# Thealexbarney/VGAudio

Measured on AMD Instinct MI355X. Metric: Msamples/s encoded (GC-ADPCM, 4096 ch) at 1/2/4/8 GPUs; % HBM roofline, higher is better.
Workload: dtype int32; 1 GPU; BASELINE configs[1]: 4096 mono channels x 48 kHz x 60 s GC-ADPCM coefficient search + encode per GPU; parallelism=units sharded x1, channels_per_gpu=4096, samples_per_channel=2880000, bit_exact_channels_checked=0

## Files before the change

vgaudio_amd/csrc/gc_encode_core.hpp:

```cpp
#pragma once
#include <cstdint>

#if defined(__HIPCC__)
#define VGA_HD __host__ __device__ __forceinline__
#else
#define VGA_HD inline
#endif

#if defined(__HIP_DEVICE_COMPILE__)
#define VGA_MUL24(a, b) __mul24((a), (b))
#define VGA_OPAQUE(v) asm("" : "+v"(v))
#define VGA_OPAQUE_S(v) asm("" : "+s"(v))
static __device__ __forceinline__ uint32_t vga_square24(int e)
{
    uint32_t r;
    asm("v_mul_i32_i24 %0, %1, %1" : "=v"(r) : "v"(e));
    return r;
}
#else
#define VGA_MUL24(a, b) ((a) * (b))
#define VGA_OPAQUE(v) ((void)0)
#define VGA_OPAQUE_S(v) ((void)0)
#endif

// ... 404 lines not shown
        const int P = (HAVE_P0 && s == 0) ? P0_b : dot2_i16(h, cpair, kacc);
        uint32_t b;
        const int d = (int)sub_borrow_u32((uint32_t)in_b[s], (uint32_t)P, b);
        const int rd = NO_ROUND ? d : round_through_f32(d);
        const int u2 = (int)((uint32_t)rd + (uint32_t)bias2 + b) >> k;
        const int q2 = med3_i32(u2, q_lo, q_hi);
        if (s & 1) {
            umax = imax(imax(umax, u_prev), u2);
            umin = imin(imin(umin, u_prev), u2);
        }
        u_prev = u2;
        if (!OV_ONLY) r.q2[s] = q2;
        const int w = (P >> 11) + (int)((uint32_t)q2 << km11);
        h = sat_pack16(w_prev, w);
        w_prev = w;
        if ((s & 1) && !OV_ONLY) {
            if (WITH_SUM) {
                const uint32_t epk = pk_sub_sat_i16(xw[s >> 1], h);
                total = dot2_i16(epk, epk, total);
            } else
                r.pairs[s >> 1] = h;
        }
    }
    r.hist_pair = h;
    const int ov = imax(imax(umax - q_hi, q_lo - umin), 0);
    r.exact = pass_b_coef_ok(c0, c1) && ov <= 12383 && (((2 * ov + 1) << (k - 11)) <= 24766);
    r.total = (uint64_t)(uint32_t)total;
    r.max_overflow = ov;
    return r;
}
VGA_HD bool pass_a_is_final(int sp_a, int ov_a) { return sp_a >= 12 || ov_a <= 1; }
template <bool NO_ROUND>
VGA_HD PassOutB final_pass_pair(const uint32_t (&xw)[7], uint32_t hist, const int (&in_b)[14], int c0, int c1, int sp_a, int sp_b,
                                int P0_b, int &ov_a, int &sp2)
{
    ov_a = pass_fast_core_b<NO_ROUND, true, false, true>(xw, hist, in_b, c0, c1, sp_a, P0_b).max_overflow;
    sp2 = pass_a_is_final(sp_a, ov_a) ? sp_a : sp_b;
    return pass_fast_core_b<NO_ROUND, true, false>(xw, hist, in_b, c0, c1, sp2, P0_b);
}
struct FrameFlags { bool fin_a, bump_a, bump_b, generic, inexact, resume; };
VGA_HD FrameFlags frame_flags(int sp_a, int sp_b, int ov_a, int ov_b, bool coef_ok)
{
    FrameFlags f;
    const bool cap_a = sp_a >= 12, cap_b = sp_b >= 12;
    const int eff_a = cap_a ? 0 : ov_a, eff_b = cap_b ? 0 : ov_b;
    f.fin_a = eff_a < 2;
    f.bump_a = !cap_a && (unsigned)ov_a > 248u;
    f.bump_b = !f.fin_a && !cap_b && (unsigned)ov_b > 248u;
    f.generic = !coef_ok || f.bump_a || f.bump_b;
    f.inexact = !f.generic && (f.fin_a ? (cap_a && (unsigned)ov_a > 3u) : (cap_b && (unsigned)ov_b > 3u));
    f.resume = !f.generic && !f.fin_a && eff_b >= 2;
    return f;
}
VGA_HD void pack_frame_mod16(const int (&q)[14], int predictor, int scale_power, uint32_t &d0, uint32_t &d1)
{
    uint32_t wa = 0, wb = 0;
#if defined(__HIP_DEVICE_COMPILE__)
#pragma unroll
#endif
    for (int s = 0; s < 14; s++) {
        if (s < 6) wa = (wa << 4) | ((uint32_t)q[s] & 15u);
        else       wb = (wb << 4) | ((uint32_t)q[s] & 15u);
    }
    const uint32_t header = (uint32_t)((predictor << 4) | (scale_power & 0xF));
    d0 = bswap32((header << 24) | wa);
    d1 = bswap32(wb);
}
VGA_HD PassOutB as_pass_b(const PassOut &r)
{
    PassOutB o;
#if defined(__HIP_DEVICE_COMPILE__)
#pragma unroll
#endif
    for (int s = 0; s < 14; s++) o.q2[s] = r.q[s];
    o.total = r.total; o.max_overflow = r.max_overflow; o.hist_pair = r.hist_pair; o.exact = r.exact;
    return o;
}
constexpr uint64_t PACKED_SUM_CAP = 1ull << 28;
VGA_HD bool needs_exact_sum(uint64_t total, bool known_exact) { return !known_exact && total >= PACKED_SUM_CAP; }
VGA_HD PassOut pass_fast_core(const int (&x)[16], uint32_t hist, const int (&in2048p)[14], int c0, int c1, int scale_power)
{
    uint32_t xw[7];
    pack_row(x, xw);
    return pass_fast_core_t<false>(xw, hist, in2048p, c0, c1, scale_power);
}
VGA_HD PassOut pass_fast_core_no_round(const int (&x)[16], uint32_t hist, const int (&in2048p)[14], int c0, int c1,
                                       int scale_power)
{
    uint32_t xw[7];
    pack_row(x, xw);
    return pass_fast_core_t<false, true>(xw, hist, in2048p, c0, c1, scale_power);
}
VGA_HD PassOut pass_fast_core_wide(const int (&x)[16], uint32_t hist, const int (&in2048p)[14], int c0, int c1,
                                   int scale_power)
{
    uint32_t xw[7];
    pack_row(x, xw);
    return pass_fast_core_t<true>(xw, hist, in2048p, c0, c1, scale_power);
}
template <bool NO_ROUND>
VGA_HD PassOut pass_fast_core_exact_sum(const int (&x)[16], const int (&in2048p)[14], int c0, int c1, int scale_power)
{
    uint32_t xw[7];
    pack_row(x, xw);
    const uint32_t hist = pack16(x[0], x[1]);
    PassOut r = pass_fast_core_t<false, NO_ROUND>(xw, hist, in2048p, c0, c1, scale_power);
// ... 94 lines not shown
```

vgaudio_amd/csrc/gc_encode_kernel.hip:

```cpp
#include "common.hpp"
#include "gc_encode_core.hpp"
#include "gcadpcm_kernels.hpp"
#include "seams.hpp"

#include <cstdio>
#include <cstdlib>

namespace vga {
namespace gc {

constexpr int DPP_QUAD_XOR1 = 0xB1;
constexpr int DPP_QUAD_XOR2 = 0x4E;
constexpr int DPP_ROW_HALF_MIRROR = 0x141;
constexpr int DPP_ROW_MIRROR = 0x140;

template <int CTRL>
__device__ __forceinline__ int dpp(int v)
{
    return __builtin_amdgcn_update_dpp(0, v, CTRL, 0xF, 0xF, true);
}

__device__ __forceinline__ unsigned umin32(unsigned a, unsigned b) { return a < b ? a : b; }

template <class Op>
__device__ __forceinline__ unsigned row16_reduce(unsigned v, Op op)
{
    v = op(v, (unsigned)dpp<DPP_QUAD_XOR1>((int)v));
    v = op(v, (unsigned)dpp<DPP_QUAD_XOR2>((int)v));
    v = op(v, (unsigned)dpp<DPP_ROW_HALF_MIRROR>((int)v));
    v = op(v, (unsigned)dpp<DPP_ROW_MIRROR>((int)v));
    return v;
}


#ifdef VGA_DEBUG_TIMESTAMPS
__device__ unsigned long long g_vga_enc_ts[1 << 16];
extern "C" int vga_debug_encode_timestamps(unsigned long long *out, int n)
{
    return (int)hipMemcpyFromSymbol(out, HIP_SYMBOL(g_vga_enc_ts), (size_t)n * sizeof(unsigned long long));
}
#endif
__device__ unsigned long long g_vga_gc_stats[8];
extern "C" int vga_testing_gc_encode_stats(unsigned long long *out8, int reset)
{
    if (hipDeviceSynchronize() != hipSuccess) return -1;
    if (out8 && hipMemcpyFromSymbol(out8, HIP_SYMBOL(g_vga_gc_stats), 8 * sizeof(unsigned long long)) != hipSuccess) return -1;
#ifdef VGA_GC_STATS
    if (out8) out8[7] = 1;
#else
    if (out8) out8[7] = 0;
#endif
    if (reset) {
        const unsigned long long zero[8] = {0, 0, 0, 0, 0, 0, 0, 0};
        if (hipMemcpyToSymbol(HIP_SYMBOL(g_vga_gc_stats), zero, sizeof zero) != hipSuccess) return -1;
    }
    return 0;
}
constexpr int SW = 2;
constexpr int ENC_THREADS = 64 * (SW + 1);
#ifndef VGA_GC_ENCODER_PRIO
#define VGA_GC_ENCODER_PRIO 3
#endif
#ifndef VGA_GC_HELPER_PRIO
#define VGA_GC_HELPER_PRIO 0
#endif
template <int CPW>
struct Lay {
    static constexpr int CS = CPW * SW;
    static constexpr int TF = 64 / CS;
};
template <int CS, int TF>
struct GcTileT {
    uint32_t xw[CS][TF][8];
    int in2048p[CS][TF][16];
    uint32_t pre[CS][TF][8];
};
typedef short short2v __attribute__((ext_vector_type(2)));
struct XW7 { uint32_t v[7]; };

#define VGA_COLD __device__ __forceinline__

VGA_COLD int prescan_sequential_cold(XW7 xs, uint32_t hist, int c0, int c1)
{
    int x[16];
    unpack_row(xs.v, hist, x);
    return prescan_sequential(x, c0, c1);
}

#ifdef VGA_GC_R05_COLD
#define VGA_COLD_OPAQUE(v) ((void)0)
#else
#define VGA_COLD_OPAQUE(v) VGA_OPAQUE(v)
#endif
struct ColdState {
    uint32_t xw[7];
    int mp[14];
    uint32_t hist;
    int c0, c1, s1;
    int generic, start, drop, wide, resume;
    int bump_a, ov_a, ov_b;
};
struct ColdOut { PassOutB r; int final_sp; int fin; int sum_exact; };
__device__ __forceinline__
ColdOut encode_frame_cold(ColdState st, PassOutB r, int final_sp, int fin)
{
    uint32_t xw[7];
    int mp[14];
#pragma unroll
    for (int i = 0; i < 7; i++) xw[i] = st.xw[i];
#pragma unroll
    for (int i = 0; i < 14; i++) mp[i] = st.mp[i];
    int sum_exact = 0;
    if (st.drop) fin = 0;
    if (__any(st.generic != 0)) {
        if (st.generic) {
            int xg[16];
            unpack_row(xw, st.hist, xg);
#pragma unroll
            for (int i = 0; i < 16; i++) VGA_COLD_OPAQUE(xg[i]);
            const int start = st.start != -100 ? st.start
                                               : (st.bump_a ? apply_bumps(st.s1, st.ov_a) : apply_bumps(st.s1 + 1, st.ov_b));
            r = as_pass_b(resume_passes(xg, st.c0, st.c1, start, final_sp));
            fin = 1;
            sum_exact = 1;
        }
    }
    if (st.wide) fin = 1;
    if (__any(st.resume != 0)) {
// ... 20 lines not shown
                    r = as_pass_b(resume_passes(xg, st.c0, st.c1, sp - 1, final_sp));
                    sum_exact = 1;
                    break;
                }
                final_sp = sp;
                if (cap || r.max_overflow <= 1) break;
            }
            fin = 1;
        }
    }
    ColdOut o;
    o.r = r;
    o.final_sp = final_sp;
    o.fin = fin;
    o.sum_exact = sum_exact;
    return o;
}

template <bool REPAIR, int CPW, bool RAGGED>
__device__ __forceinline__ void gc_encode_piece(
    const int bx, const int by,
    const int16_t *__restrict__ pcm, int64_t pcm_pitch, int nch, int total_samples, const Pieces seg,
    const int16_t *__restrict__ coefs, const int16_t *__restrict__ hist1,
    const int16_t *__restrict__ hist2, uint8_t *__restrict__ adpcm, int64_t adpcm_pitch, int16_t *__restrict__ seg_state,
    const int *__restrict__ first_open, const Ragged &rg)
{
    constexpr bool repair = REPAIR;
    constexpr int CS = Lay<CPW>::CS, TF = Lay<CPW>::TF;
    using GcTile = GcTileT<CS, TF>;
    int64_t first_frame = seg.first(by);
    int repair_piece = 0;
    if (repair) {
        int k = SEAM_OPEN_LIMIT;
        for (int g = 0; g < CS; g++) {
            const int slot = bx * CS + g;
            if (slot < nch) {
                const int c = RAGGED ? rg.order[slot] : slot;
                k = first_open[c] < k ? first_open[c] : k;
            }
        }
        if (!is_open(k)) return;
        repair_piece = k;
        first_frame = seg.first(k);
    }
    const int total_wg = RAGGED ? rg.length[rg.order[bx * CS]] : total_samples;
    if (first_frame * 14 >= total_wg) return;
    const int64_t piece_samples = repair ? (int64_t)0x7fffffff : (int64_t)seg.frames(by) * 14;
    auto piece_samples_of = [&](int total) {
        const int64_t rem = (int64_t)total - first_frame * 14;
        return (int)(rem < 0 ? 0 : (rem < piece_samples ? rem : piece_samples));
    };
    pcm += first_frame * 14;
    adpcm += first_frame * 8;
    __shared__ GcTile s_tile[2];
    __shared__ int4 s_out[2][CS][TF][4];
    __shared__ int s_ncold[SW];
    const int tid = threadIdx.x;
    const int wave = tid >> 6;
    const bool helper = wave == SW;
    const int lane = tid & 63;
    constexpr int LPC = 64 / CPW;
    int grp = helper ? lane / TF : wave * CPW + lane / LPC;
    const int l16 = lane & (LPC - 1);
    const int hfr = lane % TF;
    const int slot_raw = bx * CS + grp;
    const bool live = slot_raw < nch;
    const int slot = live ? slot_raw : nch - 1;
    const int ch = RAGGED ? rg.order[slot] : slot;
    const int16_t *src = pcm + (RAGGED ? rg.pcm_off[ch] : (int64_t)ch * pcm_pitch);
    uint8_t *dst = adpcm + (RAGGED ? rg.adpcm_off[ch] : (int64_t)ch * adpcm_pitch);

    const int sample_count = piece_samples_of(RAGGED ? rg.length[ch] : total_samples);
    const int full_frames = sample_count / 14;
    const int tail = sample_count - full_frames * 14;
    const int frames = full_frames + (tail ? 1 : 0);
    const int frames_wg = RAGGED ? (piece_samples_of(total_wg) + 13) / 14 : frames;
    const int tiles = (frames_wg + TF - 1) / TF;

    if (helper) {
        __builtin_amdgcn_s_setprio(VGA_GC_HELPER_PRIO);
        uint32_t cpk[8];
#pragma unroll
        for (int p = 0; p < 8; p++)
            cpk[p] = (uint32_t)(uint16_t)coefs[ch * 16 + 2 * p + 1] | ((uint32_t)(uint16_t)coefs[ch * 16 + 2 * p] << 16);
        auto prepare = [&](int tile) {
            const int fr = RAGGED ? imax(imin(tile * TF + hfr, frames - 1), 0) : imin(tile * TF + hfr, frames - 1);
            int in[14];
            uint32_t w[7];
            if (fr < full_frames) {
                const uint32_t *p32 = reinterpret_cast<const uint32_t *>(src + (int64_t)fr * 14);
#pragma unroll
                for (int i = 0; i < 7; i++) w[i] = p32[i];
#pragma unroll
                for (int i = 0; i < 7; i++) {
                    in[2 * i] = (int)(int16_t)(w[i] & 0xFFFF);
                    in[2 * i + 1] = (int)w[i] >> 16;
                }
            } else {
#pragma unroll
                for (int s = 0; s < 14; s++) in[s] = (s < tail) ? (int)src[(int64_t)fr * 14 + s] : 0;
#pragma unroll
                for (int i = 0; i < 7; i++) w[i] = (uint32_t)(in[2 * i] & 0xFFFF) | ((uint32_t)in[2 * i + 1] << 16);
            }
            GcTile &T = s_tile[tile & 1];
            uint4 *xr = reinterpret_cast<uint4 *>(&T.xw[grp][hfr][0]);
            xr[0] = make_uint4(w[0], w[1], w[2], w[3]);
            xr[1] = make_uint4(w[4], w[5], w[6], 0u);
            int4 *qr = reinterpret_cast<int4 *>(&T.in2048p[grp][hfr][0]);
            qr[0] = make_int4(pass_b_row(in[0]), pass_b_row(in[1]), pass_b_row(in[2]), pass_b_row(in[3]));
            qr[1] = make_int4(pass_b_row(in[4]), pass_b_row(in[5]), pass_b_row(in[6]), pass_b_row(in[7]));
            qr[2] = make_int4(pass_b_row(in[8]), pass_b_row(in[9]), pass_b_row(in[10]), pass_b_row(in[11]));
            qr[3] = make_int4(pass_b_row(in[12]), pass_b_row(in[13]), 0, 0);
            uint32_t pair[12];
#pragma unroll
            for (int k = 0; k < 12; k++)
                pair[k] = (k & 1) ? __builtin_amdgcn_alignbit(w[(k + 1) / 2], w[(k - 1) / 2], 16) : w[k / 2];
            uint32_t pre[8];
#pragma unroll
            for (int p = 0; p < 8; p++) {
                int dmax = 0, dmin = 0;
#ifdef VGA_GC_ABLATE_HELPER_PRESCAN
                dmax = in[2 + p] & 1023;
                dmin = -(in[3 + p] & 1023);
#else
#pragma unroll
                for (int k = 0; k < 12; k++) {
                    const int predicted = div2048(__builtin_amdgcn_sdot2(__builtin_bit_cast(short2v, pair[k]),
                                                                         __builtin_bit_cast(short2v, cpk[p]), 0, false));
                    const int d = in[k + 2] - predicted;
                    dmax = imax(dmax, d);
                    dmin = imin(dmin, d);
                }
#endif
                pre[p] = (uint32_t)(clamp16i(dmax) & 0xFFFF) | ((uint32_t)clamp16i(dmin) << 16);
            }
            uint4 *pr = reinterpret_cast<uint4 *>(&T.pre[grp][hfr][0]);
            pr[0] = make_uint4(pre[0], pre[1], pre[2], pre[3]);
            pr[1] = make_uint4(pre[4], pre[5], pre[6], pre[7]);
        };
        auto flush = [&](int tile) {
            const int fr = tile * TF + hfr;
            if (!live || fr >= frames) return;
            const int4 *rec = &s_out[tile & 1][grp][hfr][0];
            const int4 r0 = rec[0], r1 = rec[1], r2 = rec[2], r3 = rec[3];
            const int q[14] = {r0.x, r0.y, r0.z, r0.w, r1.x, r1.y, r1.z, r1.w, r2.x, r2.y, r2.z, r2.w, r3.x, r3.y};
            uint2 v;
            pack_frame_mod16(q, r3.z, r3.w, v.x, v.y);
            if (fr < full_frames) {
                *reinterpret_cast<uint2 *>(dst + (int64_t)fr * 8) = v;
            } else {
                const int nbytes = (tail + 2 + 1) / 2;
                const uint64_t both = ((uint64_t)v.y << 32) | v.x;
                for (int b = 0; b < nbytes; b++) dst[(int64_t)fr * 8 + b] = (uint8_t)(both >> (8 * b));
            }
        };
        if (tiles > 0) prepare(0);
        __syncthreads();
        for (int tile = 0; tile < tiles; tile++) {
            if (tile + 1 < tiles) prepare(tile + 1);
            if (tile > 0) flush(tile - 1);
            __syncthreads();
        }
        if (tiles > 0) flush(tiles - 1);
        return;
    }

    __builtin_amdgcn_s_setprio(VGA_GC_ENCODER_PRIO);
    int p = CPW == 4 ? l16 >> 1 : l16;
    const bool cand_b = CPW == 4 && (l16 & 1) != 0;
    const int c0 = coefs[ch * 16 + 2 * p];
    const int c1 = coefs[ch * 16 + 2 * p + 1];
    const bool coef_ok = pass_b_coef_ok(c0, c1);
    int h0 = hist2 ? hist2[ch] : 0;
    int h1 = hist1 ? hist1[ch] : 0;
    if (repair) {
        h0 = seg_state[((int64_t)(repair_piece - 1) * nch + ch) * 2];
        h1 = seg_state[((int64_t)(repair_piece - 1) * nch + ch) * 2 + 1];
    } else if (by > 0 && (!RAGGED || frames > 0)) {
        h0 = src[-2];
        h1 = src[-1];
    }
    uint32_t hpk = pack16(h0, h1);

    if (lane == 0) s_ncold[wave] = 0;
    struct Row { uint32_t xw[7]; int mp[14]; uint32_t pre; };
    auto read_row = [&](const GcTile &T, int j, Row &R) {
        const uint4 *xr = reinterpret_cast<const uint4 *>(&T.xw[grp][j][0]);
        const uint4 a0 = xr[0], a1 = xr[1];
        asm volatile("" ::"v"(a1.w));
        uint32_t *xw = R.xw;
        xw[0] = a0.x; xw[1] = a0.y; xw[2] = a0.z; xw[3] = a0.w; xw[4] = a1.x; xw[5] = a1.y; xw[6] = a1.z;
        const int4 *qr = reinterpret_cast<const int4 *>(&T.in2048p[grp][j][0]);
        const int4 e0 = qr[0], e1 = qr[1], e2 = qr[2], e3 = qr[3];
        asm volatile("" ::"v"(e3.z), "v"(e3.w));
        int *mp = R.mp;
        mp[0] = e0.x; mp[1] = e0.y; mp[2] = e0.z; mp[3] = e0.w; mp[4] = e1.x; mp[5] = e1.y; mp[6] = e1.z; mp[7] = e1.w;
        mp[8] = e2.x; mp[9] = e2.y; mp[10] = e2.z; mp[11] = e2.w; mp[12] = e3.x; mp[13] = e3.y;
        R.pre = T.pre[grp][j][p];
    };
    auto pack = [](const uint32_t (&xw)[7]) {
        XW7 xs;
#pragma unroll
        for (int i = 0; i < 7; i++) xs.v[i] = xw[i];
        return xs;
    };
    const uint32_t cpk = pack16(c1, c0);
    auto wide_total = [&](const uint32_t (&xw)[7], const int (&mp)[14], int sp) -> uint64_t {
        int row[14];
#pragma unroll
        for (int i = 0; i < 14; i++) row[i] = mp[i] - PASS_B_OFF;
        return pass_fast_core_wide(xw, hpk, row, c0, c1, sp).total;
    };
    const bool head_numer = __builtin_amdgcn_ballot_w64(!coef_ok) == 0;
    auto prescan_head = [&](const Row &R, int &d0, int &d1, int &P0) __attribute__((always_inline)) {
        P0 = predicted_b(hpk, cpk);
        if (__builtin_expect(head_numer, 1)) {
            d0 = head_distance_numer_b(R.mp[0], P0);
            d1 = head_distance_numer_b(R.mp[1], predicted_b(__builtin_amdgcn_alignbit(R.xw[0], hpk, 16), cpk));
        } else {
            d0 = pair_lo(R.xw[0]) - div2048(dot2_i16_wrap(hpk, cpk));
            d1 = pair_hi(R.xw[0]) - div2048(dot2_i16_wrap(__builtin_amdgcn_alignbit(R.xw[0], hpk, 16), cpk));
        }
    };
    auto first_scale = [&](const Row &R, int d0, int d1) __attribute__((always_inline)) -> int {
        const int dmax = imax(imax((int)(int16_t)(R.pre & 0xFFFF), d0), d1);
        const int dmin = imin(imin((int)R.pre >> 16, d0), d1);
        int sum, pos;
        int s1 = first_scale_power_nt(dmax, dmin, sum, pos);
        if (__builtin_expect(__builtin_amdgcn_ballot_w64(sum == 0) != 0, 0)) {
            if (sum == 0 && first_scale_tie(pos)) s1 = first_scale_power_from_md(prescan_sequential_cold(pack(R.xw), hpk, c0, c1));
        }
        return s1;
    };

    auto encode_frame = [&](Row &R, int buf, int j, bool upd) {
        const uint32_t (&xw)[7] = R.xw;
        int s1, P0;
        {
            int d0, d1;
            prescan_head(R, d0, d1, P0);
            s1 = first_scale(R, d0, d1);
        }
        int final_sp = imin(s1 + (cand_b ? 1 : 0), 12);
        const bool at_cap = final_sp >= 12;
        const unsigned ov_limit = at_cap ? 3u : 248u;
        PassOutB r = pass_fast_core_b<false, true>(xw, hpk, R.mp, c0, c1, final_sp, P0);
        const bool rare = !coef_ok || (!at_cap && (unsigned)r.max_overflow > ov_limit);
        const int eff = at_cap ? 0 : r.max_overflow;
        const int eff_other = dpp<DPP_QUAD_XOR1>(eff);
        bool fin = eff < 2 && (eff_other | (cand_b ? 0 : 2)) >= 2;
        const bool resume = !cand_b && imin(eff, eff_other) >= 2;
        const bool inexact = fin && at_cap && (unsigned)r.max_overflow > ov_limit;
        constexpr unsigned SAT = (1u << 28) - 1;
        auto argmin32 = [&](const PassOutB &r, bool fin, bool &sat) __attribute__((always_inline)) -> int {
            const unsigned tot = umin32((unsigned)(r.total >> 32) ? SAT : (unsigned)r.total, SAT);
            const unsigned key = fin ? ((tot << 4) | (unsigned)l16) : 0xFFFFFFFFu;
            const unsigned best = row16_reduce(key, [](unsigned a, unsigned b) { return a < b ? a : b; });
            sat = __any((best >> 4) >= SAT);
            return (int)(best & 15u);
        };
        auto argmin64 = [&](uint64_t total, bool fin) __attribute__((always_inline)) -> int {
            uint64_t key = fin ? ((total << 4) | (uint64_t)l16) : ~0ull;
#define VGA_MIN64_STAGE(CTRL)                                                          \
            {                                                                          \
                const unsigned olo = (unsigned)dpp<CTRL>((int)(uint32_t)key);          \
                const unsigned ohi = (unsigned)dpp<CTRL>((int)(uint32_t)(key >> 32));  \
                const uint64_t okey = ((uint64_t)ohi << 32) | olo;                     \
                key = okey < key ? okey : key;                                         \
            }
            VGA_MIN64_STAGE(DPP_QUAD_XOR1)
            VGA_MIN64_STAGE(DPP_QUAD_XOR2)
            VGA_MIN64_STAGE(DPP_ROW_HALF_MIRROR)
            VGA_MIN64_STAGE(DPP_ROW_MIRROR)
#undef VGA_MIN64_STAGE
            return (int)(key & 15u);
        };
        auto commit = [&](const PassOutB &r, int final_sp, int winner) __attribute__((always_inline)) {
            const bool won = l16 == winner;
            const unsigned pay = row16_reduce(won ? r.hist_pair : 0u,
                                              [](unsigned a, unsigned b) { return a | b; });
            if (won) {
                int4 *rec = &s_out[buf][grp][j][0];
                rec[0] = make_int4(r.q2[0], r.q2[1], r.q2[2], r.q2[3]);
                rec[1] = make_int4(r.q2[4], r.q2[5], r.q2[6], r.q2[7]);
                rec[2] = make_int4(r.q2[8], r.q2[9], r.q2[10], r.q2[11]);
                rec[3] = make_int4(r.q2[12], r.q2[13], p, final_sp);
            }
            if (!RAGGED || upd) hpk = pay;
        };
        bool sat = false;
        const int winner32 = argmin32(r, fin && !inexact, sat);
        if (__builtin_expect(__any(rare || resume || inexact) || sat, 0)) {
#ifdef VGA_GC_STATS
            if (lane == 0) atomicAdd(&s_ncold[wave], 1);
#endif
            ColdState st;
#pragma unroll
            for (int i = 0; i < 7; i++) st.xw[i] = xw[i];
#pragma unroll
            for (int i = 0; i < 14; i++) st.mp[i] = R.mp[i];
            st.hist = hpk;
            st.c0 = c0; st.c1 = c1; st.s1 = s1;
            const bool redo = __any(rare);
            st.generic = redo && !cand_b; st.start = s1 - 1; st.drop = redo && cand_b;
            st.wide = !redo && inexact; st.resume = !redo && resume;
            st.bump_a = 0; st.ov_a = 0; st.ov_b = 0;
            const ColdOut o = encode_frame_cold(st, r, final_sp, fin);
            bool sat2 = false;
            int winner = argmin32(o.r, o.fin != 0, sat2);
            if (sat2) {
                uint64_t total = o.r.total;
                if (o.fin != 0 && needs_exact_sum(total, o.sum_exact != 0))
                    total = wide_total(xw, R.mp, o.final_sp);
                winner = argmin64(total, o.fin != 0);
            }
            commit(o.r, o.final_sp, winner);
        } else
            commit(r, final_sp, winner32);
    };

    auto encode_frame8 = [&](Row &R, int buf, int j, bool upd) {
        const uint32_t (&xw)[7] = R.xw;
        int s1, P0;
        {
            int d0, d1;
            prescan_head(R, d0, d1, P0);
            s1 = first_scale(R, d0, d1);
        }
        const int sp_a = imin(s1, 12), sp_b = imin(s1 + 1, 12);
        PassOutB r;
        int ov_a, sp2;
#ifdef VGA_GC_NO_FAST_PASSES
        bool short_passes = false;
#else
        bool short_passes = !__any(sp_b > 9);
#endif
        if (short_passes) {
            r = final_pass_pair<true>(xw, hpk, R.mp, c0, c1, sp_a, sp_b, P0, ov_a, sp2);
            const bool trusted = !coef_ok || (pass_no_round_is_exact(sp_a, ov_a) && pass_no_round_is_exact(sp2, r.max_overflow));
            short_passes = !__any(!trusted);
        }
        if (!short_passes) r = final_pass_pair<false>(xw, hpk, R.mp, c0, c1, sp_a, sp_b, P0, ov_a, sp2);
        const int ov_2 = r.max_overflow;
        const FrameFlags ff = frame_flags(sp_a, sp_b, ov_a, ov_2, coef_ok);
        const bool bump_a = ff.bump_a, generic = ff.generic, inexact = ff.inexact;
#ifdef VGA_GC_ABLATE_THIRD_TRIPS
        const bool resume = false;
#else
        const bool resume = ff.resume;
#endif
        r.total = error_sum_pairs(xw, r.pairs);
        r.exact = true;
        const int final_sp = sp2;
        constexpr unsigned SAT = (1u << 28) - 1;
        auto argmin32 = [&](const PassOutB &r, bool fin, bool &sat) __attribute__((always_inline)) -> int {
            const unsigned tot = umin32((unsigned)(r.total >> 32) ? SAT : (unsigned)r.total, SAT);
            unsigned key = fin ? ((tot << 3) | (unsigned)p) : 0xFFFFFFFFu;
            key = umin32(key, (unsigned)dpp<DPP_QUAD_XOR1>((int)key));
            key = umin32(key, (unsigned)dpp<DPP_QUAD_XOR2>((int)key));
            key = umin32(key, (unsigned)dpp<DPP_ROW_HALF_MIRROR>((int)key));
            sat = __any((key >> 3) >= SAT);
            return (int)(key & 7u);
        };
        auto argmin64 = [&](uint64_t total, bool fin) __attribute__((always_inline)) -> int {
            uint64_t key = fin ? ((total << 3) | (uint64_t)p) : ~0ull;
#define VGA_MIN64_STAGE(CTRL)                                                          \
            {                                                                          \
                const unsigned olo = (unsigned)dpp<CTRL>((int)(uint32_t)key);          \
                const unsigned ohi = (unsigned)dpp<CTRL>((int)(uint32_t)(key >> 32));  \
                const uint64_t okey = ((uint64_t)ohi << 32) | olo;                     \
                key = okey < key ? okey : key;                                         \
            }
            VGA_MIN64_STAGE(DPP_QUAD_XOR1)
            VGA_MIN64_STAGE(DPP_QUAD_XOR2)
            VGA_MIN64_STAGE(DPP_ROW_HALF_MIRROR)
#undef VGA_MIN64_STAGE
            return (int)(key & 7u);
        };
        auto commit = [&](const PassOutB &r, int final_sp, int winner) __attribute__((always_inline)) {
            const bool won = p == winner;
            unsigned pay = won ? r.hist_pair : 0u;
            pay |= (unsigned)dpp<DPP_QUAD_XOR1>((int)pay);
            pay |= (unsigned)dpp<DPP_QUAD_XOR2>((int)pay);
            pay |= (unsigned)dpp<DPP_ROW_HALF_MIRROR>((int)pay);
            if (won) {
                int4 *rec = &s_out[buf][grp][j][0];
                rec[0] = make_int4(r.q2[0], r.q2[1], r.q2[2], r.q2[3]);
                rec[1] = make_int4(r.q2[4], r.q2[5], r.q2[6], r.q2[7]);
                rec[2] = make_int4(r.q2[8], r.q2[9], r.q2[10], r.q2[11]);
                rec[3] = make_int4(r.q2[12], r.q2[13], p, final_sp);
            }
            if (!RAGGED || upd) hpk = pay;
        };
        bool sat = false;
        const int winner32 = argmin32(r, !(generic || resume || inexact), sat);
        if (__builtin_expect(__any(generic || resume || inexact) || sat, 0)) {
#ifdef VGA_GC_STATS
            if (lane == 0) atomicAdd(&s_ncold[wave], 1);
#endif
            ColdState st;
#pragma unroll
            for (int i = 0; i < 7; i++) st.xw[i] = xw[i];
#pragma unroll
            for (int i = 0; i < 14; i++) st.mp[i] = R.mp[i];
            st.hist = hpk;
            st.c0 = c0; st.c1 = c1; st.s1 = s1;
            st.generic = generic; st.drop = 0; st.wide = inexact; st.resume = resume;
#ifdef VGA_GC_R05_COLD
            st.start = !coef_ok ? s1 - 1 : (bump_a ? apply_bumps(s1, ov_a) : apply_bumps(s1 + 1, ov_2));
#else
            st.start = !coef_ok ? s1 - 1 : -100;
#endif
            st.bump_a = bump_a; st.ov_a = ov_a; st.ov_b = ov_2;
            const ColdOut o = encode_frame_cold(st, r, final_sp, (generic || resume) ? 0 : 1);
            bool sat2 = false;
            int winner = argmin32(o.r, o.fin != 0, sat2);
            if (sat2) {
                uint64_t total = o.r.total;
                if (o.fin != 0 && needs_exact_sum(total, o.sum_exact != 0))
                    total = wide_total(xw, R.mp, o.final_sp);
                winner = argmin64(total, o.fin != 0);
            }
            commit(o.r, o.final_sp, winner);
        } else
            commit(r, final_sp, winner32);
    };
    auto encode_one = [&](Row &R, int buf, int j, bool upd) __attribute__((always_inline)) {
        if constexpr (CPW == 4) encode_frame(R, buf, j, upd);
        else encode_frame8(R, buf, j, upd);
    };

#ifdef VGA_DEBUG_TIMESTAMPS
    if (!repair && tid == 0 && gridDim.y != 1) g_vga_enc_ts[2 * ((blockIdx.y * gridDim.x + blockIdx.x) & 32767)] = wall_clock64();
#endif
    __syncthreads();
    for (int tile = 0; tile < tiles; tile++) {
        const int buf = tile & 1;
        const int nf = imin(TF, frames_wg - tile * TF);
        const int left = frames - tile * TF;
#ifndef VGA_GC_NO_TILE_REDERIVE
        {
            int l = lane;
            asm volatile("" : "+v"(l));
            grp = wave * CPW + l / LPC;
            p = CPW == 4 ? (l & (LPC - 1)) >> 1 : (l & (LPC - 1));
        }
#endif
        const GcTile &T = s_tile[buf];
        Row RA, RB;
        read_row(T, 0, RA);
#pragma unroll 1
        for (int j = 0; j < nf; j += 2) {
            read_row(T, imin(j + 1, TF - 1), RB);
            encode_one(RA, buf, j, j < left);
            if (j + 1 < nf) {
                read_row(T, imin(j + 2, TF - 1), RA);
                encode_one(RB, buf, j + 1, j + 1 < left);
            }
        }
        __syncthreads();
    }
    if (seg_state && !repair && live && l16 == 0) {
        int16_t *st = seg_state + ((int64_t)by * nch + ch) * 2;
        st[0] = (int16_t)pair_lo(hpk);
        st[1] = (int16_t)pair_hi(hpk);
    }
    if (lane == 0) {
        atomicAdd(&g_vga_gc_stats[3], (unsigned long long)frames_wg);
        atomicAdd(&g_vga_gc_stats[4], (unsigned long long)s_ncold[wave]);
        if (wave == 0) atomicAdd(&g_vga_gc_stats[6], 1ull);
    }
#ifdef VGA_DEBUG_TIMESTAMPS
    if (!repair && tid == 0 && gridDim.y != 1) g_vga_enc_ts[2 * ((blockIdx.y * gridDim.x + blockIdx.x) & 32767) + 1] = wall_clock64();
#endif
}


template <bool REPAIR, int CPW, bool RAGGED>
__global__ __launch_bounds__(ENC_THREADS) __attribute__((amdgpu_waves_per_eu(3, 3))) void gc_encode_kernel(
    const int16_t *__restrict__ pcm, int64_t pcm_pitch, int nch, int total_samples, const Pieces seg,
    const int16_t *__restrict__ coefs, const int16_t *__restrict__ hist1,
    const int16_t *__restrict__ hist2, uint8_t *__restrict__ adpcm, int64_t adpcm_pitch, int16_t *__restrict__ seg_state,
    const int *__restrict__ first_open, const Ragged rg)
{
    gc_encode_piece<REPAIR, CPW, RAGGED>(blockIdx.x, blockIdx.y, pcm, pcm_pitch, nch, total_samples, seg, coefs, hist1, hist2, adpcm,
                                         adpcm_pitch, seg_state, first_open, rg);
}

__device__ __forceinline__ void store_frame_bytes(uint8_t *dst, uint32_t d0, uint32_t d1, int nbytes)
{
    const uint64_t bits = ((uint64_t)d1 << 32) | d0;
    for (int b = 0; b < nbytes; b++) dst[b] = (uint8_t)(bits >> (8 * b));
}

template <int LPC>
__device__ __forceinline__ void seam_run(const int16_t *__restrict__ src, uint8_t *__restrict__ dst, int c0, int c1, bool coef_ok,
                                         int pr, int ch, int k, int64_t f0, int total_samples, int piece_frames, int max_frames, int force_open,
                                         int &h0, int &h1, int g2, int g1, bool &open, int &frames_run)
{
    static_assert(LPC == 8 || LPC == 16, "a lane per predictor, or per (predictor, candidate)");
    const bool cand_b = LPC == 16 && (threadIdx.x & 1) != 0;
    const int full_frames = total_samples / 14;
    const int64_t f_end = imin((int)imin((int)(f0 + piece_frames), (int)(f0 + max_frames)), full_frames);
    const int64_t f_last = full_frames > 0 ? full_frames - 1 : 0;
    auto fetch = [&](int64_t f, uint32_t (&w)[7], uint2 &old) {
        const int64_t fc = f < f_last ? f : f_last;
        const uint32_t *p32 = reinterpret_cast<const uint32_t *>(src + fc * 14);
#pragma unroll
        for (int i = 0; i < 7; i++) w[i] = p32[i];
        old = *reinterpret_cast<const uint2 *>(dst + fc * 8);
// ... 183 lines not shown
        const int nibbles = tail + 2;
        store_frame_bytes(dst + (int64_t)full_frames * 8, d0, d1, nibbles / 2 + (nibbles & 1));
    }
}

template <int LPC>
__device__ __forceinline__ void seam_piece(
    const int slot_raw, const int k, const int lane,
    const int16_t *__restrict__ pcm, int64_t pcm_pitch, int nch, int total_samples, const Pieces seg,
    const int16_t *__restrict__ coefs, uint8_t *adpcm, int64_t adpcm_pitch,
    const int16_t *seg_state, int *first_open, int *seam_flag, int *seam_end, int force_open, const Ragged &rg)
{
    const int pr = LPC == 16 ? (lane >> 1) & 7 : lane & 7;
    const bool lead = (lane & (LPC - 1)) == 0;
    const int64_t f0 = seg.first(k);
    const int slot = slot_raw < nch ? slot_raw : nch - 1;
    const int ch = rg.order ? rg.order[slot] : slot;
    if (rg.order) total_samples = rg.length[ch];
    const bool valid = slot_raw < nch && f0 * 14 < total_samples;
    const int16_t *src = pcm + (rg.order ? rg.pcm_off[ch] : (int64_t)ch * pcm_pitch);
    uint8_t *dst = adpcm + (rg.order ? rg.adpcm_off[ch] : (int64_t)ch * adpcm_pitch);
    const int16_t *cf = coefs + ch * 16;
    const int c0 = cf[2 * pr], c1 = cf[2 * pr + 1];
    const bool coef_ok = (c0 < 0 ? -c0 : c0) + (c1 < 0 ? -c1 : c1) <= 32767;
    int h0 = valid ? seg_state[((int64_t)(k - 1) * nch + ch) * 2] : 0;
    int h1 = valid ? seg_state[((int64_t)(k - 1) * nch + ch) * 2 + 1] : 0;
    const int g2 = valid ? src[f0 * 14 - 2] : 0, g1 = valid ? src[f0 * 14 - 1] : 0;
    bool open = valid;
    int frames_run = 0;
    seam_run<LPC>(src, dst, c0, c1, coef_ok, pr, ch, k, f0, total_samples, seg.frames(k), seg.frames(k), force_open, h0, h1, g2, g1, open, frames_run);
    if (valid && lead) {
        atomicAdd(&g_vga_gc_stats[open ? 1 : 0], 1ull);
        atomicAdd(&g_vga_gc_stats[2], (unsigned long long)frames_run);
        seam_flag[(int64_t)(k - 1) * nch + ch] = open ? 1 : 0;
        if (open) {
            seam_end[(int64_t)(k - 1) * nch + ch] = (int)(((unsigned)h1 << 16) | ((unsigned)h0 & 0xFFFFu));
            atomicMin(&first_open[ch], k);
        }
    }
}

template <int LPC>
__global__ __launch_bounds__(64) void gc_encode_seam_kernel(
    const int16_t *__restrict__ pcm, int64_t pcm_pitch, int nch, int total_samples, const Pieces seg,
    const int16_t *__restrict__ coefs, uint8_t *__restrict__ adpcm, int64_t adpcm_pitch,
    const int16_t *__restrict__ seg_state, int *__restrict__ first_open, int *__restrict__ seam_flag,
    int *__restrict__ seam_end, int force_open, const Ragged rg)
{
    seam_piece<LPC>(blockIdx.x * (64 / LPC) + (threadIdx.x / LPC), blockIdx.y + 1, threadIdx.x, pcm, pcm_pitch, nch, total_samples, seg, coefs, adpcm,
               adpcm_pitch, seg_state, first_open, seam_flag, seam_end, force_open, rg);
}

template <int CPW, bool RAGGED>
__global__ __launch_bounds__(ENC_THREADS) __attribute__((amdgpu_waves_per_eu(3, 3))) void gc_encode_persistent_kernel(
    const int16_t *__restrict__ pcm, int64_t pcm_pitch, int nch, int total_samples, const Pieces seg,
    const int16_t *__restrict__ coefs, const int16_t *__restrict__ hist1,
    const int16_t *__restrict__ hist2, uint8_t *adpcm, int64_t adpcm_pitch, int16_t *seg_state,
    const Ragged rg, int groups, int segments, int *__restrict__ queue, int *__restrict__ seam_count, int *first_open,
    int *seam_flag, int *seam_end, int force_open)
{
    static_assert(CPW == 8, "the seams inside the persistent kernel use the (channel, predictor) layout");
    constexpr int CS = Lay<CPW>::CS;
    __shared__ int s_item;
    __shared__ int s_seam[2];
    const int items = RAGGED && rg.items ? rg.n_items : groups * segments;
#ifdef VGA_DEBUG_TIMESTAMPS
    if (threadIdx.x == 0) g_vga_enc_ts[2 * (blockIdx.x & 32767)] = wall_clock64();
#endif
    for (;;) {
        if (threadIdx.x == 0) s_item = atomicAdd(queue, 1);
        __syncthreads();
        const int item = s_item;
        __syncthreads();
        if (item >= items) {
#ifdef VGA_DEBUG_TIMESTAMPS
            if (threadIdx.x == 0) g_vga_enc_ts[2 * (blockIdx.x & 32767) + 1] = wall_clock64();
#endif
            return;
        }
        int g = item % groups, y = item / groups;
        if (RAGGED && rg.items) {
            const uint32_t v = rg.items[item];
            g = (int)(v & 0xFFFFFu);
            y = (int)(v >> 20);
        }
        gc_encode_piece<false, CPW, RAGGED>(g, y, pcm, pcm_pitch, nch, total_samples, seg, coefs, hist1, hist2, adpcm, adpcm_pitch,
                                            seg_state, (const int *)nullptr, rg);
        if (segments <= 1) continue;
        __threadfence();
        __syncthreads();
        if (threadIdx.x == 0) {
            const int total_wg = RAGGED ? rg.length[rg.order[g * CS]] : total_samples;
            auto exists = [&](int piece) { return piece < segments && seg.first(piece) * 14 < total_wg; };
            int at_start = 0, at_end = 0;
            if (exists(y)) {
                if (y >= 1 && atomicAdd(&seam_count[(int64_t)(y - 1) * groups + g], 1) == 1) at_start = y;
                if (exists(y + 1) && atomicAdd(&seam_count[(int64_t)y * groups + g], 1) == 1) at_end = y + 1;
            }
            s_seam[0] = at_start;
            s_seam[1] = at_end;
        }
        __syncthreads();
        const int seam_a = s_seam[0], seam_b = s_seam[1];
        if ((seam_a | seam_b) != 0) {
            __threadfence();
            const int wave = threadIdx.x >> 6, lane = threadIdx.x & 63;
            if (wave < SW) {
// ... 41 lines not shown
    int last_k = 0;
    for (int k = kmin; k < segments; k++) {
        const int64_t f0 = seg.first(k);
        const bool exists = f0 * 14 < total_samples;
        if (!__any(exists)) break;
        last_k = k;
        const bool is_last = seg.first(k + 1) * 14 >= total_samples || k == segments - 1;
        const int64_t idx = (int64_t)(k - 1) * nch + ch;
        const bool flagged = live && exists && seam_flag[idx] != 0;
        const int ended = seam_end[idx];
        const bool ran = live && have && exists;
        bool open = ran;
        int h0 = v0, h1 = v1;
        if (__any(ran)) {
            const int g2 = seg_state[idx * 2], g1 = seg_state[idx * 2 + 1];
            if (ran && lead && is_last) {
                seg_state[idx * 2] = (int16_t)v0;
                seg_state[idx * 2 + 1] = (int16_t)v1;
            }
            seam_run<LPC>(src, dst, c0, c1, coef_ok, pr, ch, k, f0, total_samples, seg.frames(k), seg.frames(k), force_open, h0, h1, g2, g1, open, frames_run);
        }
        if (!exists) {
        } else if (ran && open) {
            v0 = h0;
            v1 = h1;
        } else if (flagged) {
            have = true;
            v0 = (int)(int16_t)(ended & 0xFFFF);
            v1 = ended >> 16;
        } else
            have = false;
    }
    if (__any(live && have && total_samples % 14 != 0))
        encode_tail_frame<LPC>(src, dst, c0, c1, coef_ok, pr, total_samples, v0, v1, live && have && total_samples % 14 != 0);
    (void)last_k;
    if (live && lead && frames_run) atomicAdd(&g_vga_gc_stats[2], (unsigned long long)frames_run);
    if (live && lead) first_open[ch] = SEAM_NONE;
}

constexpr int MIN_PIECE_FRAMES = 3584;

constexpr int RAGGED_OVERSUBSCRIPTION = 4;
constexpr int PERSISTENT_MIN_GROUPS_FACTOR = 32;
constexpr int PERSISTENT_SCHEDULE_GROUPS_FACTOR = 8;
constexpr int PERSISTENT_ITEMS_PER_WORKGROUP = 4;
constexpr int PERSISTENT_BIG_ROUNDS = 3;
constexpr int PERSISTENT_SMALL_ROUNDS = 2;
constexpr int PERSISTENT_SMALL_FRAMES = 4096;
constexpr int MAX_PIECES = 1024;

static int persistent_wgs_per_cu()
{
#ifdef VGA_TUNING
    if (const char *e = std::getenv("VGA_HIP_GC_WGS_PER_CU")) return imin(imax(std::atoi(e), 1), 4);
#endif
    return 4;
}

int plan_encode_pieces(int groups, int frames, int64_t group_frames, bool ragged, bool *persistent_out, Pieces *seg_out, int layout)
{
    return plan_encode_pieces_on(device_cu_count(), groups, frames, group_frames, ragged, persistent_out, seg_out, layout);
}

int plan_encode_pieces_on(int cus, int groups, int frames, int64_t group_frames, bool ragged, bool *persistent_out, Pieces *seg_out, int layout)
{
    const int pmode = encoder_persistent_mode();
    const bool persistent = layout != 4 && (pmode == 2 || (pmode == 0 && (ragged || groups * PERSISTENT_MIN_GROUPS_FACTOR >= cus * 4)));
    int segments = cus * 4 / (groups > 0 ? groups : 1);
    if (persistent && (pmode == 2 || ragged)) segments = (cus * 4 * PERSISTENT_ITEMS_PER_WORKGROUP + groups - 1) / groups;
    if (ragged) {
        const int64_t want = (int64_t)cus * 4 * (persistent ? PERSISTENT_ITEMS_PER_WORKGROUP : RAGGED_OVERSUBSCRIPTION);
        int64_t piece = (group_frames + want - 1) / want;
        if (piece < MIN_PIECE_FRAMES) piece = MIN_PIECE_FRAMES;
        segments = (int)((frames + piece - 1) / piece);
    }
    if (segments > frames / MIN_PIECE_FRAMES) segments = frames / MIN_PIECE_FRAMES;
    if (segments < 1) segments = 1;
    if (segments > MAX_PIECES) segments = MAX_PIECES;
    if (encoder_segments_override() > 0) segments = imin(imin(imax(frames / 64, 1), encoder_segments_override()), MAX_PIECES);
    Pieces seg;
    seg.big = (frames + segments - 1) / segments;
    seg.nb = segments;
    seg.small = seg.big;
    if (persistent && encoder_segments_override() <= 0 && frames >= 4 * MIN_PIECE_FRAMES &&
        (ragged || groups * PERSISTENT_SCHEDULE_GROUPS_FACTOR >= cus * 4)) {
        int big_rounds = ragged ? PERSISTENT_BIG_ROUNDS + 1 : PERSISTENT_BIG_ROUNDS, small_rounds = PERSISTENT_SMALL_ROUNDS, small = PERSISTENT_SMALL_FRAMES;
#ifdef VGA_TUNING
        if (const char *e = std::getenv("VGA_HIP_GC_SCHEDULE")) std::sscanf(e, "%d,%d,%d", &big_rounds, &small_rounds, &small);
#endif
        small = imax(small, MIN_PIECE_FRAMES);
        big_rounds = imax(big_rounds, 1);
        const int wgs = cus * persistent_wgs_per_cu();
        const int64_t per_wg = group_frames / wgs + 1;
        int ns = (small_rounds * wgs + groups / 2) / groups;
        if ((int64_t)ns * small > frames / 2) ns = frames / (2 * small);
        int big = (int)imax((int)((per_wg - (int64_t)small_rounds * small) / big_rounds), small);
        int nb = (int)((frames - (int64_t)ns * small + big - 1) / big);
        if (nb < 1) nb = 1;
        if (!ragged) big = (int)((frames - (int64_t)ns * small + nb - 1) / nb);
        if (big < small) big = small;
        seg.big = big;
        seg.nb = nb;
        seg.small = small;
        segments = nb + ns;
        while (segments > 1 && seg.first(segments - 1) >= frames) segments--;
        if (segments > MAX_PIECES) {
            segments = MAX_PIECES;
// ... 131 lines not shown
```

Baseline: 80350 Msamples/s.

## Interleave per-frame shared tile slots and defer cold-path flag computation

Restructures the shared-memory tile from separate xw/in2048p/pre/out arrays into per-frame Slot structs, with the output record inside the slot and padding per group. The frame loop walks slot pointers and loads the per-predictor pre value separately, and a valid-frame marker is stored in xw[7] for the ragged case. A cheaper frame_goes_cold predicate replaces the full frame_flags on the hot path, and the full flags are now computed only inside the cold branch. Lane and wave indices are re-derived with mbcnt and readfirstlane so they stay scalar. These changes aim to cut LDS address arithmetic, bank conflicts and hot-path ALU work, at the risk of a different shared-memory footprint and more register pressure.

```diff
diff --git a/vgaudio_amd/csrc/gc_encode_core.hpp b/vgaudio_amd/csrc/gc_encode_core.hpp
--- a/vgaudio_amd/csrc/gc_encode_core.hpp
+++ b/vgaudio_amd/csrc/gc_encode_core.hpp
@@ -480,6 +480,17 @@
     f.resume = !f.generic && !f.fin_a && eff_b >= 2;
     return f;
 }
+VGA_HD int frame_flag_limit(int sp) { return sp >= 12 ? 3 : 1; }
+struct FrameCold { bool cold, fin_a; };
+VGA_HD FrameCold frame_goes_cold(int sp_a, int sp_b, int ov_a, int ov_2, bool coef_ok)
+{
+    const bool cap_a = sp_a >= 12;
+    const bool a_bad = ov_a > frame_flag_limit(sp_a), b_bad = ov_2 > frame_flag_limit(sp_b);
+    FrameCold f;
+    f.fin_a = cap_a | !a_bad;
+    f.cold = !coef_ok | (a_bad & (cap_a | (ov_a > 248) | b_bad));
+    return f;
+}
 VGA_HD void pack_frame_mod16(const int (&q)[14], int predictor, int scale_power, uint32_t &d0, uint32_t &d1)
 {
     uint32_t wa = 0, wb = 0;
diff --git a/vgaudio_amd/csrc/gc_encode_kernel.hip b/vgaudio_amd/csrc/gc_encode_kernel.hip
--- a/vgaudio_amd/csrc/gc_encode_kernel.hip
+++ b/vgaudio_amd/csrc/gc_encode_kernel.hip
@@ -63,6 +63,9 @@
 #endif
 #ifndef VGA_GC_HELPER_PRIO
 #define VGA_GC_HELPER_PRIO 0
+#endif
+#ifndef VGA_GC_PERSISTENT_WAVES_PER_EU
+#define VGA_GC_PERSISTENT_WAVES_PER_EU 3, 3
 #endif
 template <int CPW>
 struct Lay {
@@ -71,9 +74,14 @@
 };
 template <int CS, int TF>
 struct GcTileT {
-    uint32_t xw[CS][TF][8];
-    int in2048p[CS][TF][16];
-    uint32_t pre[CS][TF][8];
+    struct Slot {
+        uint32_t xw[8];
+        int in2048p[16];
+        uint32_t pre[8];
+        int4 out[4];
+    };
+    struct Group { Slot f[TF]; uint32_t pad[4]; };
+    Group g[CS];
 };
 typedef short short2v __attribute__((ext_vector_type(2)));
 struct XW7 { uint32_t v[7]; };
@@ -200,8 +208,11 @@
     };
     pcm += first_frame * 14;
     adpcm += first_frame * 8;
-    __shared__ GcTile s_tile[2];
-    __shared__ int4 s_out[2][CS][TF][4];
+    using Slot = typename GcTile::Slot;
+    static_assert(TF % 2 == 0, "the frame loop takes a tile's frames in pairs");
+    struct Tiles { GcTile t[2]; Slot end; };
+    __shared__ Tiles s_tiles;
+    GcTile (&s_tile)[2] = s_tiles.t;
     __shared__ int s_ncold[SW];
     const int tid = threadIdx.x;
     const int wave = tid >> 6;
@@ -250,11 +261,11 @@
 #pragma unroll
                 for (int i = 0; i < 7; i++) w[i] = (uint32_t)(in[2 * i] & 0xFFFF) | ((uint32_t)in[2 * i + 1] << 16);
             }
-            GcTile &T = s_tile[tile & 1];
-            uint4 *xr = reinterpret_cast<uint4 *>(&T.xw[grp][hfr][0]);
+            Slot &T = s_tile[tile & 1].g[grp].f[hfr];
+            uint4 *xr = reinterpret_cast<uint4 *>(&T.xw[0]);
             xr[0] = make_uint4(w[0], w[1], w[2], w[3]);
-            xr[1] = make_uint4(w[4], w[5], w[6], 0u);
-            int4 *qr = reinterpret_cast<int4 *>(&T.in2048p[grp][hfr][0]);
+            xr[1] = make_uint4(w[4], w[5], w[6], (!RAGGED || tile * TF + hfr < frames) ? 1u : 0u);
+            int4 *qr = reinterpret_cast<int4 *>(&T.in2048p[0]);
             qr[0] = make_int4(pass_b_row(in[0]), pass_b_row(in[1]), pass_b_row(in[2]), pass_b_row(in[3]));
             qr[1] = make_int4(pass_b_row(in[4]), pass_b_row(in[5]), pass_b_row(in[6]), pass_b_row(in[7]));
             qr[2] = make_int4(pass_b_row(in[8]), pass_b_row(in[9]), pass_b_row(in[10]), pass_b_row(in[11]));
@@ -282,14 +293,14 @@
 #endif
                 pre[p] = (uint32_t)(clamp16i(dmax) & 0xFFFF) | ((uint32_t)clamp16i(dmin) << 16);
             }
-            uint4 *pr = reinterpret_cast<uint4 *>(&T.pre[grp][hfr][0]);
+            uint4 *pr = reinterpret_cast<uint4 *>(&T.pre[0]);
             pr[0] = make_uint4(pre[0], pre[1], pre[2], pre[3]);
             pr[1] = make_uint4(pre[4], pre[5], pre[6], pre[7]);
         };
         auto flush = [&](int tile) {
             const int fr = tile * TF + hfr;
             if (!live || fr >= frames) return;
-            const int4 *rec = &s_out[tile & 1][grp][hfr][0];
+            const int4 *rec = &s_tile[tile & 1].g[grp].f[hfr].out[0];
             const int4 r0 = rec[0], r1 = rec[1], r2 = rec[2], r3 = rec[3];
             const int q[14] = {r0.x, r0.y, r0.z, r0.w, r1.x, r1.y, r1.z, r1.w, r2.x, r2.y, r2.z, r2.w, r3.x, r3.y};
             uint2 v;
@@ -314,6 +325,7 @@
     }
 
     __builtin_amdgcn_s_setprio(VGA_GC_ENCODER_PRIO);
+    const int wave_u = __builtin_amdgcn_readfirstlane(wave);
     int p = CPW == 4 ? l16 >> 1 : l16;
     const bool cand_b = CPW == 4 && (l16 & 1) != 0;
     const int c0 = coefs[ch * 16 + 2 * p];
@@ -331,20 +343,28 @@
     uint32_t hpk = pack16(h0, h1);
 
     if (lane == 0) s_ncold[wave] = 0;
-    struct Row { uint32_t xw[7]; int mp[14]; uint32_t pre; };
-    auto read_row = [&](const GcTile &T, int j, Row &R) {
-        const uint4 *xr = reinterpret_cast<const uint4 *>(&T.xw[grp][j][0]);
+    struct Row { uint32_t xw[7]; int mp[14]; };
+    auto read_row = [&](const Slot &T, Row &R) {
+        const uint4 *xr = reinterpret_cast<const uint4 *>(&T.xw[0]);
         const uint4 a0 = xr[0], a1 = xr[1];
         asm volatile("" ::"v"(a1.w));
         uint32_t *xw = R.xw;
         xw[0] = a0.x; xw[1] = a0.y; xw[2] = a0.z; xw[3] = a0.w; xw[4] = a1.x; xw[5] = a1.y; xw[6] = a1.z;
-        const int4 *qr = reinterpret_cast<const int4 *>(&T.in2048p[grp][j][0]);
+        const int4 *qr = reinterpret_cast<const int4 *>(&T.in2048p[0]);
         const int4 e0 = qr[0], e1 = qr[1], e2 = qr[2], e3 = qr[3];
         asm volatile("" ::"v"(e3.z), "v"(e3.w));
         int *mp = R.mp;
         mp[0] = e0.x; mp[1] = e0.y; mp[2] = e0.z; mp[3] = e0.w; mp[4] = e1.x; mp[5] = e1.y; mp[6] = e1.z; mp[7] = e1.w;
         mp[8] = e2.x; mp[9] = e2.y; mp[10] = e2.z; mp[11] = e2.w; mp[12] = e3.x; mp[13] = e3.y;
-        R.pre = T.pre[grp][j][p];
+    };
+    auto read_pre = [&](const Slot &T) __attribute__((always_inline)) -> uint32_t {
+        int pp = p;
+        asm volatile("" : "+v"(pp));
+        return T.pre[pp];
+    };
+    auto slot_has_frame = [&](const Slot &T) __attribute__((always_inline)) -> bool {
+        if constexpr (RAGGED) return T.xw[7] != 0u;
+        else return true;
     };
     auto pack = [](const uint32_t (&xw)[7]) {
         XW7 xs;
@@ -370,9 +390,9 @@
             d1 = pair_hi(R.xw[0]) - div2048(dot2_i16_wrap(__builtin_amdgcn_alignbit(R.xw[0], hpk, 16), cpk));
         }
     };
-    auto first_scale = [&](const Row &R, int d0, int d1) __attribute__((always_inline)) -> int {
-        const int dmax = imax(imax((int)(int16_t)(R.pre & 0xFFFF), d0), d1);
-        const int dmin = imin(imin((int)R.pre >> 16, d0), d1);
+    auto first_scale = [&](const Row &R, uint32_t pre, int d0, int d1) __attribute__((always_inline)) -> int {
+        const int dmax = imax(imax((int)(int16_t)(pre & 0xFFFF), d0), d1);
+        const int dmin = imin(imin((int)pre >> 16, d0), d1);
         int sum, pos;
         int s1 = first_scale_power_nt(dmax, dmin, sum, pos);
         if (__builtin_expect(__builtin_amdgcn_ballot_w64(sum == 0) != 0, 0)) {
@@ -381,13 +401,13 @@
         return s1;
     };
 
-    auto encode_frame = [&](Row &R, int buf, int j, bool upd) {
+    auto encode_frame = [&](Row &R, Slot &S, uint32_t pre) {
         const uint32_t (&xw)[7] = R.xw;
         int s1, P0;
         {
             int d0, d1;
             prescan_head(R, d0, d1, P0);
-            s1 = first_scale(R, d0, d1);
+            s1 = first_scale(R, pre, d0, d1);
         }
         int final_sp = imin(s1 + (cand_b ? 1 : 0), 12);
         const bool at_cap = final_sp >= 12;
@@ -428,13 +448,13 @@
             const unsigned pay = row16_reduce(won ? r.hist_pair : 0u,
                                               [](unsigned a, unsigned b) { return a | b; });
             if (won) {
-                int4 *rec = &s_out[buf][grp][j][0];
+                int4 *rec = &S.out[0];
                 rec[0] = make_int4(r.q2[0], r.q2[1], r.q2[2], r.q2[3]);
                 rec[1] = make_int4(r.q2[4], r.q2[5], r.q2[6], r.q2[7]);
                 rec[2] = make_int4(r.q2[8], r.q2[9], r.q2[10], r.q2[11]);
                 rec[3] = make_int4(r.q2[12], r.q2[13], p, final_sp);
             }
-            if (!RAGGED || upd) hpk = pay;
+            if (slot_has_frame(S)) hpk = pay;
         };
         bool sat = false;
         const int winner32 = argmin32(r, fin && !inexact, sat);
@@ -467,13 +487,13 @@
             commit(r, final_sp, winner32);
     };
 
-    auto encode_frame8 = [&](Row &R, int buf, int j, bool upd) {
+    auto encode_frame8 = [&](Row &R, Slot &S, uint32_t pre) {
         const uint32_t (&xw)[7] = R.xw;
         int s1, P0;
         {
             int d0, d1;
             prescan_head(R, d0, d1, P0);
-            s1 = first_scale(R, d0, d1);
+            s1 = first_scale(R, pre, d0, d1);
         }
         const int sp_a = imin(s1, 12), sp_b = imin(s1 + 1, 12);
         PassOutB r;
@@ -490,12 +510,11 @@
         }
         if (!short_passes) r = final_pass_pair<false>(xw, hpk, R.mp, c0, c1, sp_a, sp_b, P0, ov_a, sp2);
         const int ov_2 = r.max_overflow;
-        const FrameFlags ff = frame_flags(sp_a, sp_b, ov_a, ov_2, coef_ok);
-        const bool bump_a = ff.bump_a, generic = ff.generic, inexact = ff.inexact;
 #ifdef VGA_GC_ABLATE_THIRD_TRIPS
-        const bool resume = false;
+        const FrameFlags ff0 = frame_flags(sp_a, sp_b, ov_a, ov_2, coef_ok);
+        const bool cold = ff0.generic || ff0.inexact;
 #else
-        const bool resume = ff.resume;
+        const bool cold = frame_goes_cold(sp_a, sp_b, ov_a, ov_2, coef_ok).cold;
 #endif
         r.total = error_sum_pairs(xw, r.pairs);
         r.exact = true;
@@ -532,19 +551,26 @@
             pay |= (unsigned)dpp<DPP_QUAD_XOR2>((int)pay);
             pay |= (unsigned)dpp<DPP_ROW_HALF_MIRROR>((int)pay);
             if (won) {
-                int4 *rec = &s_out[buf][grp][j][0];
+                int4 *rec = &S.out[0];
                 rec[0] = make_int4(r.q2[0], r.q2[1], r.q2[2], r.q2[3]);
                 rec[1] = make_int4(r.q2[4], r.q2[5], r.q2[6], r.q2[7]);
                 rec[2] = make_int4(r.q2[8], r.q2[9], r.q2[10], r.q2[11]);
                 rec[3] = make_int4(r.q2[12], r.q2[13], p, final_sp);
             }
-            if (!RAGGED || upd) hpk = pay;
+            if (slot_has_frame(S)) hpk = pay;
         };
         bool sat = false;
-        const int winner32 = argmin32(r, !(generic || resume || inexact), sat);
-        if (__builtin_expect(__any(generic || resume || inexact) || sat, 0)) {
+        const int winner32 = argmin32(r, !cold, sat);
+        if (__builtin_expect(__builtin_amdgcn_ballot_w64(cold) != 0 || sat, 0)) {
 #ifdef VGA_GC_STATS
             if (lane == 0) atomicAdd(&s_ncold[wave], 1);
+#endif
+            const FrameFlags ff = frame_flags(sp_a, sp_b, ov_a, ov_2, coef_ok);
+            const bool bump_a = ff.bump_a, generic = ff.generic, inexact = ff.inexact;
+#ifdef VGA_GC_ABLATE_THIRD_TRIPS
+            const bool resume = false;
+#else
+            const bool resume = ff.resume;
 #endif
             ColdState st;
 #pragma unroll
@@ -573,9 +599,9 @@
         } else
             commit(r, final_sp, winner32);
     };
-    auto encode_one = [&](Row &R, int buf, int j, bool upd) __attribute__((always_inline)) {
-        if constexpr (CPW == 4) encode_frame(R, buf, j, upd);
-        else encode_frame8(R, buf, j, upd);
+    auto encode_one = [&](Row &R, Slot &S, uint32_t pre) __attribute__((always_inline)) {
+        if constexpr (CPW == 4) encode_frame(R, S, pre);
+        else encode_frame8(R, S, pre);
     };
 
 #ifdef VGA_DEBUG_TIMESTAMPS
@@ -585,25 +611,27 @@
     for (int tile = 0; tile < tiles; tile++) {
         const int buf = tile & 1;
         const int nf = imin(TF, frames_wg - tile * TF);
-        const int left = frames - tile * TF;
 #ifndef VGA_GC_NO_TILE_REDERIVE
         {
-            int l = lane;
-            asm volatile("" : "+v"(l));
-            grp = wave * CPW + l / LPC;
+            unsigned zero = 0;
+            asm volatile("" : "+s"(zero));
+            const int l = (int)__builtin_amdgcn_mbcnt_hi(~0u, __builtin_amdgcn_mbcnt_lo(~0u, zero));
+            grp = wave_u * CPW + l / LPC;
             p = CPW == 4 ? (l & (LPC - 1)) >> 1 : (l & (LPC - 1));
         }
 #endif
-        const GcTile &T = s_tile[buf];
+        Slot *S = &s_tile[buf].g[grp].f[0];
         Row RA, RB;
-        read_row(T, 0, RA);
+        read_row(S[0], RA);
 #pragma unroll 1
-        for (int j = 0; j < nf; j += 2) {
-            read_row(T, imin(j + 1, TF - 1), RB);
-            encode_one(RA, buf, j, j < left);
+        for (int j = 0; j < nf; j += 2, S += 2) {
+            const uint32_t pre_a = read_pre(S[0]);
+            read_row(S[1], RB);
+            encode_one(RA, S[0], pre_a);
             if (j + 1 < nf) {
-                read_row(T, imin(j + 2, TF - 1), RA);
-                encode_one(RB, buf, j + 1, j + 1 < left);
+                const uint32_t pre_b = read_pre(S[1]);
+                read_row(S[2], RA);
+                encode_one(RB, S[1], pre_b);
             }
         }
         __syncthreads();
@@ -893,7 +921,7 @@
 }
 
 template <int CPW, bool RAGGED>
-__global__ __launch_bounds__(ENC_THREADS) __attribute__((amdgpu_waves_per_eu(3, 3))) void gc_encode_persistent_kernel(
+__global__ __launch_bounds__(ENC_THREADS) __attribute__((amdgpu_waves_per_eu(VGA_GC_PERSISTENT_WAVES_PER_EU))) void gc_encode_persistent_kernel(
     const int16_t *__restrict__ pcm, int64_t pcm_pitch, int nch, int total_samples, const Pieces seg,
     const int16_t *__restrict__ coefs, const int16_t *__restrict__ hist1,
     const int16_t *__restrict__ hist2, uint8_t *adpcm, int64_t adpcm_pitch, int16_t *seg_state,
@@ -1041,7 +1069,7 @@
 static int persistent_wgs_per_cu()
 {
 #ifdef VGA_TUNING
-    if (const char *e = std::getenv("VGA_HIP_GC_WGS_PER_CU")) return imin(imax(std::atoi(e), 1), 4);
+    if (const char *e = std::getenv("VGA_HIP_GC_WGS_PER_CU")) return imin(imax(std::atoi(e), 1), 5);
 #endif
     return 4;
 }
```

New measurement: 82050 Msamples/s, median of 6. +2.1%, better.
